# facebookresearch/pytorchvideo

Measured on NVIDIA H100. Metric: clips/sec forward (synthetic 3xTx224^2), higher is better.
Workload: dtype f16

## Files before the change

### pytorchvideo_b200/csrc/pv_epilogue.cuh

```cuda
#pragma once
#include "pv_common.cuh"
#include "pv_sm90.cuh"

namespace pv {
namespace sm90 {

constexpr int EPI_STAGING_BYTES = 2 * 128 * 128;
constexpr int EPI_THREADS = 256;
constexpr int EPI_BAR_ID = 1;
constexpr int MAX_BN = 128;

struct EpiParams {
  CUtensorMap y_map;
  CUtensorMap r_map;
  int block_n, Co, rows, act, has_residual;
  const __half* addend;
  long long add_n, add_t;
  int add_off;
  int o_ext[4], o_box[4], o_pos[4];
  int hw, To;
};

inline void epi_set_addend(EpiParams& E, const pv_conv3d_desc* d) {
  E.addend = static_cast<const __half*>(d->addend);
  E.add_n = d->add_n_stride;
  E.add_t = d->add_t_stride;
  E.add_off = d->add_ch_off;
  E.hw = d->Ho * d->Wo;
  E.To = d->To;
}

__device__ __forceinline__ void tma_store_5d(const void* tmap, uint32_t src, int c0, int c1, int c2, int c3,
                                             int c4) {
  asm volatile(
      "cp.async.bulk.tensor.5d.global.shared::cta.bulk_group [%0, {%2, %3, %4, %5, %6}], [%1];" ::"l"(
          reinterpret_cast<uint64_t>(tmap)),
      "r"(src), "r"(c0), "r"(c1), "r"(c2), "r"(c3), "r"(c4)
      : "memory");
}
__device__ __forceinline__ void tma_store_commit() { asm volatile("cp.async.bulk.commit_group;" ::: "memory"); }
__device__ __forceinline__ void tma_store_wait_read0() { asm volatile("cp.async.bulk.wait_group.read 0;" ::: "memory"); }
__device__ __forceinline__ void tma_store_wait_all() { asm volatile("cp.async.bulk.wait_group 0;" ::: "memory"); }
__device__ __forceinline__ void fence_proxy_async_smem() { asm volatile("fence.proxy.async.shared::cta;" ::: "memory"); }
__device__ __forceinline__ void epi_bar_sync(int id, int nthreads) {
  asm volatile("bar.sync %0, %1;" ::"r"(id), "r"(nthreads) : "memory");
}

template <int ACT>
__device__ __forceinline__ float act_t(float x) {
  if (ACT == PV_ACT_RELU) return fmaxf(x, 0.f);
  if (ACT == PV_ACT_NONE) return x;
  return apply_act(x, ACT);
}

__device__ __forceinline__ void epilogue_begin(const EpiParams& E, uint32_t staging, uint32_t res_bar, int n0, int c1,
                                               int c2, int c3, int c4) {
  tma_store_wait_read0();
  if (E.has_residual) {
    const int nsub = (E.block_n + 63) >> 6;
    mbar_arrive_expect_tx(res_bar, (uint32_t)(nsub * E.rows * 128));
    for (int s = 0; s < nsub; ++s)
      tma_load_5d(staging + (uint32_t)s * 16384u, &E.r_map, res_bar, n0 + s * 64, c1, c2, c3, c4);
  }
}

template <int BN, int ACT, bool RES>
__device__ __forceinline__ void epi_math(const float (&d)[BN / 2], uint8_t* stg, const float* __restrict__ scale,
                                         const float* __restrict__ bias, int Co, int n0, int ctid) {
  const int lane = ctid & 31;
  const int row0 = 64 * (ctid >> 7) + 16 * ((ctid >> 5) & 3) + (lane >> 2);
  const int cq = 2 * (lane & 3);
#pragma unroll
  for (int j = 0; j < BN / 8; ++j) {
    const int col = 8 * j + cq;
    const int c = n0 + col;
    float2 s = make_float2(0.f, 0.f), b = make_float2(0.f, 0.f);
    if (c < Co) {
      s = __ldg(reinterpret_cast<const float2*>(scale + c));
      b = __ldg(reinterpret_cast<const float2*>(bias + c));
    }
#pragma unroll
    for (int i = 0; i < 2; ++i) {
      const int row = row0 + 8 * i;
      __half2* cell = reinterpret_cast<__half2*>(stg + (col >> 6) * 16384 + row * 128 +
                                                 ((((col & 63) >> 3) ^ (row & 7)) << 4) + cq * 2);
      float f0 = fmaf(d[4 * j + 2 * i], s.x, b.x), f1 = fmaf(d[4 * j + 2 * i + 1], s.y, b.y);
// ... 30 lines not shown
      const unsigned v = (unsigned)(m == 0 ? c1 : m == 1 ? c2 : m == 2 ? c3 : c4) + r % (unsigned)E.o_box[m];
      r /= (unsigned)E.o_box[m];
      inside &= v < (unsigned)E.o_ext[m];
      pos += v * (unsigned)E.o_pos[m];
    }
    if (!inside) continue;
    const unsigned nt = pos / (unsigned)E.hw;
    const unsigned n = nt / (unsigned)E.To, t = nt - n * (unsigned)E.To;
    const uint4 av = __ldg(reinterpret_cast<const uint4*>(acol + n * E.add_n + t * E.add_t));
    uint4* cell = reinterpret_cast<uint4*>(stg + (col >> 6) * 16384 + row * 128 + ((((col & 63) >> 3) ^ (row & 7)) << 4));
    uint4 sv = *cell;
    __half2* s2 = reinterpret_cast<__half2*>(&sv);
    const __half2* a2 = reinterpret_cast<const __half2*>(&av);
#pragma unroll
    for (int k = 0; k < 4; ++k) {
      const float2 f = __half22float2(s2[k]), g = __half22float2(a2[k]);
      s2[k] = __floats2half2_rn(f.x + g.x, f.y + g.y);
    }
    *cell = sv;
  }
}

template <int BN>
__device__ __forceinline__ void epilogue_tile(const EpiParams& E, const float* __restrict__ scale,
                                              const float* __restrict__ bias, const float (&d)[BN / 2],
                                              uint32_t staging, uint8_t* staging_gen, uint32_t res_bar,
                                              uint32_t& res_phase, int ctid, int n0, int c1, int c2, int c3, int c4) {
  epi_bar_sync(EPI_BAR_ID, EPI_THREADS);
  if (E.has_residual) {
    mbar_wait(res_bar, res_phase);
    res_phase ^= 1u;
  }
  switch (E.act) {
    case PV_ACT_RELU: epi_math_res<BN, PV_ACT_RELU>(E.has_residual, d, staging_gen, scale, bias, E.Co, n0, ctid); break;
    case PV_ACT_NONE: epi_math_res<BN, PV_ACT_NONE>(E.has_residual, d, staging_gen, scale, bias, E.Co, n0, ctid); break;
    case PV_ACT_SWISH: epi_math_res<BN, PV_ACT_SWISH>(E.has_residual, d, staging_gen, scale, bias, E.Co, n0, ctid); break;
    case PV_ACT_GELU: epi_math_res<BN, PV_ACT_GELU>(E.has_residual, d, staging_gen, scale, bias, E.Co, n0, ctid); break;
    default: epi_math_res<BN, PV_ACT_SIGMOID>(E.has_residual, d, staging_gen, scale, bias, E.Co, n0, ctid); break;
  }
  if (E.addend) {
    epi_bar_sync(EPI_BAR_ID, EPI_THREADS);
    epi_addend<BN>(E, staging_gen, ctid, n0, c1, c2, c3, c4);
  }
  fence_proxy_async_smem();
  epi_bar_sync(EPI_BAR_ID, EPI_THREADS);
  if (ctid == 0) {
    const int nsub = (E.block_n + 63) >> 6;
    for (int s = 0; s < nsub; ++s) tma_store_5d(&E.y_map, staging + (uint32_t)s * 16384u, n0 + s * 64, c1, c2, c3, c4);
    tma_store_commit();
  }
}

__host__ __device__ inline int round_block_n(int co) { return co <= 16 ? 16 : (co <= 32 ? 32 : (co <= 64 ? 64 : 128)); }

}
}
```

### pytorchvideo_b200/csrc/pv_igemm.cu

```cuda
#include "pv_common.cuh"
#include "pv_sm90.cuh"
#include "pv_epilogue.cuh"

#include <mutex>
#include <stdlib.h>
#include <string.h>

namespace pv {

using namespace sm90;

constexpr int IG_BM = 128;
constexpr int IG_MAX_TAPS = 64;
constexpr int IG_MAX_MAPS = 8;
constexpr int IG_PROD_WARPS = 4;
constexpr int IG_CONS_WARPS = 8;
constexpr int IG_THREADS = (IG_CONS_WARPS + IG_PROD_WARPS) * 32;

struct IgemmParams {
  CUtensorMap a_maps[IG_MAX_MAPS];
  CUtensorMap b_map;
  int O[4];
  int box[4];
  int nt[4];
  int rows;
  int n_tiles, m_tiles;
  int block_n;
  int Co;
  int taps, num_kc;
  int kbytes;
  int stages;
  int G, cpt;
  int split_ab;
  EpiParams epi;
  signed char tap_q[IG_MAX_TAPS][4];
  unsigned char tap_map[IG_MAX_TAPS];
};

template <int BN, int KB, bool GROUPED>
__device__ __forceinline__ void igemm_body(const IgemmParams& P, const float* __restrict__ scale,
                                           const float* __restrict__ bias, int span_tiles) {
  extern __shared__ uint8_t smem_raw[];
  const uint32_t smem_base = (smem_u32(smem_raw) + 1023u) & ~1023u;
  uint8_t* smem_gen = smem_raw + (smem_base - smem_u32(smem_raw));
  const int stages = P.stages;
  constexpr int G = 128 / KB, K16 = KB / 32;
  const uint32_t a_bytes = (uint32_t)IG_BM * KB;
  const uint32_t b_bytes = (uint32_t)BN * KB;
  const uint32_t stage_bytes = (uint32_t)G * (a_bytes + b_bytes);
  constexpr int k_elems = KB / 2;
  const uint32_t staging_off = (uint32_t)((stages * stage_bytes + 1023u) & ~1023u);
  const uint32_t staging = smem_base + staging_off;
  const uint32_t bar_base = staging + (uint32_t)EPI_STAGING_BYTES;
  auto full_bar = [&](int s) { return bar_base + 8u * s; };
  auto empty_bar = [&](int s) { return bar_base + 8u * (stages + s); };
  const uint32_t res_bar = bar_base + 8u * (2 * stages);

  const int warp = threadIdx.x >> 5;
  const int lane = threadIdx.x & 31;

  if (threadIdx.x == 0) {
    prefetch_tmap(&P.b_map);
    prefetch_tmap(&P.a_maps[0]);
    prefetch_tmap(&P.epi.y_map);
    for (int s = 0; s < stages; ++s) {
      mbar_init(full_bar(s), 1);
      mbar_init(empty_bar(s), IG_CONS_WARPS);
    }
    mbar_init(res_bar, 1);
    fence_mbar_init();
  }
  __syncthreads();
  asm volatile("griddepcontrol.wait;" ::: "memory");
  asm volatile("griddepcontrol.launch_dependents;" ::: "memory");

  const int total_tiles = P.n_tiles * P.m_tiles;
  const int num_kb = P.taps * P.num_kc;
  auto tile_coords = [&](int tile, int& n_tile, int (&o)[4]) {
    n_tile = tile % P.n_tiles;
    int mt = tile / P.n_tiles;
#pragma unroll
    for (int i = 0; i < 4; ++i) { o[i] = (mt % P.nt[i]) * P.box[i]; mt /= P.nt[i]; }
  };

  if (warp >= IG_CONS_WARPS) {
    const int pw = warp - IG_CONS_WARPS;
    const int nsplit = P.split_ab;
    if (pw < nsplit) {
      int stage = 0;
      uint32_t phase = 0;
      const uint32_t tx_bytes = (uint32_t)P.rows * KB + b_bytes;
      const int num_kc = P.num_kc, cpt = P.cpt;
      for (int tile = blockIdx.x; tile < total_tiles; tile += gridDim.x) {
        int n_tile, o[4];
        tile_coords(tile, n_tile, o);
        const int n0 = n_tile * BN;
        const int c0 = GROUPED ? (n_tile / span_tiles) * num_kc * k_elems : 0;
        int tap = 0, kc = 0;
        for (int ch = 0; ch < cpt; ++ch) {
          const int kb0 = ch * G;
          const int nsub = min(G, num_kb - kb0);
          mbar_wait(empty_bar(stage), phase ^ 1u);
          const uint32_t st_base = smem_base + (uint32_t)stage * stage_bytes;
          if (elect_one()) {
            if (pw == 0) mbar_arrive_expect_tx(full_bar(stage), (uint32_t)G * tx_bytes);
            int tp = tap, kk = kc;
            for (int j = 0; j < G; ++j) {
              const bool pad = j >= nsub;
              const int t = pad ? P.taps - 1 : tp;
              if ((2 * j) % nsplit == pw) {
                const void* amap = &P.a_maps[P.tap_map[t]];
                tma_load_5d(st_base + (uint32_t)j * a_bytes, amap, full_bar(stage),
                            (pad ? num_kc * k_elems : kk * k_elems) + c0,
                            o[0] + P.tap_q[t][0], o[1] + P.tap_q[t][1], o[2] + P.tap_q[t][2], o[3] + P.tap_q[t][3]);
              }
              if ((2 * j + 1) % nsplit == pw)
                tma_load_2d(st_base + (uint32_t)G * a_bytes + (uint32_t)j * b_bytes, &P.b_map, full_bar(stage),
                            (kb0 + j) * k_elems, n0);
              if (++kk == num_kc) { kk = 0; ++tp; }
            }
          }
          __syncwarp();
          for (int j = 0; j < nsub; ++j) { if (++kc == num_kc) { kc = 0; ++tap; } }
          if (++stage == stages) { stage = 0; phase ^= 1u; }
        }
      }
    }
  } else {
    const int ctid = threadIdx.x;
    const uint32_t a_row_off = (uint32_t)(ctid >> 7) * 64u * (uint32_t)KB;
    const int cpt = P.cpt;
    int stage = 0;
    uint32_t phase = 0, res_phase = 0;
    float acc[BN / 2];
#pragma unroll
    for (int i = 0; i < BN / 2; ++i) acc[i] = 0.f;
    for (int tile = blockIdx.x; tile < total_tiles; tile += gridDim.x) {
      int n_tile, o[4];
      tile_coords(tile, n_tile, o);
      if (ctid == 0) epilogue_begin(P.epi, staging, res_bar, n_tile * BN, o[0], o[1], o[2], o[3]);
      int prev = -1;
      for (int ch = 0; ch < cpt; ++ch) {
        mbar_wait(full_bar(stage), phase);
        const uint32_t st_base = smem_base + (uint32_t)stage * stage_bytes;
        acc_fence(acc);
        wgmma_fence();
#pragma unroll
        for (int j = 0; j < G; ++j) {
          const uint64_t a_desc = make_kmajor_desc(st_base + (uint32_t)j * a_bytes + a_row_off, KB);
          const uint64_t b_desc = make_kmajor_desc(st_base + (uint32_t)G * a_bytes + (uint32_t)j * b_bytes, KB);
#pragma unroll
          for (int k = 0; k < K16; ++k) {
            Wgmma<BN>::mma(acc, a_desc + (uint64_t)(2 * k), b_desc + (uint64_t)(2 * k), (ch | j | k) != 0 ? 1u : 0u);
          }
        }
        wgmma_commit();
        acc_fence(acc);
        wgmma_wait<1>();
        mbar_arrive_if(empty_bar(prev < 0 ? stage : prev), prev >= 0 && lane == 0);
        prev = stage;
        if (++stage == stages) { stage = 0; phase ^= 1u; }
      }
      wgmma_wait<0>();
      acc_fence(acc);
      mbar_arrive_if(empty_bar(prev < 0 ? stage : prev), prev >= 0 && lane == 0);
      epilogue_tile<BN>(P.epi, scale, bias, acc, staging, smem_gen + staging_off, res_bar, res_phase, ctid, n_tile * BN,
                        o[0], o[1], o[2], o[3]);
    }
    if (ctid == 0) tma_store_wait_all();
  }
}

template <int BN, int KB>
__global__ void __launch_bounds__(IG_THREADS, 1)
conv3d_igemm_kernel(const __grid_constant__ IgemmParams P, const float* __restrict__ scale,
                    const float* __restrict__ bias) {
  igemm_body<BN, KB, false>(P, scale, bias, 1);
}

template <int BN, int KB>
__global__ void __launch_bounds__(IG_THREADS, 1)
conv3d_igemm_grouped_kernel(const __grid_constant__ IgemmParams P, const float* __restrict__ scale,
                            const float* __restrict__ bias, int span_tiles) {
  igemm_body<BN, KB, true>(P, scale, bias, span_tiles);
}

typedef CUresult (*EncodeTiledFn)(CUtensorMap*, CUtensorMapDataType, cuuint32_t, void*,
                                  const cuuint64_t*, const cuuint64_t*, const cuuint32_t*,
                                  const cuuint32_t*, CUtensorMapInterleave, CUtensorMapSwizzle,
                                  CUtensorMapL2promotion, CUtensorMapFloatOOBfill);

EncodeTiledFn get_encode_fn() {
// ... 197 lines not shown
      if (grouped && (c < 64 || span_n % c)) continue;
      if (c > round_block_n(co16)) continue;
      if (c < co16 && (c % 64)) continue;
      const long long tiles = (long long)P.m_tiles * cdiv(d->Co, c);
      const double waves = (double)cdiv(tiles, sm_count);
      const double cost = waves * tile_cycles(c) + 1e-3 * cdiv(d->Co, c);
      if (cost < best) { best = cost; bn = c; }
    }
    P.block_n = bn;
    P.n_tiles = (int)cdiv(d->Co, bn);
  }
  const bool wmode = window_mode(d);
  const bool narrow = conv3d_tma_narrow(d);
  const int win = wmode ? window_elems(d) : (narrow ? d->Ci : 64);
  P.kbytes = 2 * win;
  P.Co = d->Co;
  P.taps = wmode ? d->kt * d->kh : d->kt * d->kh * d->kw;
  P.num_kc = (wmode || narrow) ? 1 : d->ci_pad64 / 64;
  P.epi.block_n = P.block_n;
  P.epi.Co = d->Co;
  P.epi.rows = P.rows;
  P.epi.act = d->act;
  P.epi.has_residual = d->has_residual;
  epi_set_addend(P.epi, d);
  const int kb_bytes = (IG_BM + P.block_n) * P.kbytes;
  const size_t smem_fixed = 2048  + EPI_STAGING_BYTES + 16;
  {
    const int num_kb = P.taps * P.num_kc;
    const int G = 128 / P.kbytes;
    const int budget = (int)(227 * 1024 - smem_fixed) - 8 * (2 * 24 + 1);
    int st = budget / (G * kb_bytes);
    if (st > 24 / G) st = 24 / G > 2 ? 24 / G : 2;
    if (st < 2) st = 2;
    P.G = G;
    P.split_ab = G >= 2 ? 4 : 2;
    P.cpt = (num_kb + G - 1) / G;
    P.stages = st;
    if (grouped && (G != 1 || P.block_n > span_n || span_n % P.block_n)) {
      set_error("internal: grouped mode needs one k-block per stage and BLOCK_N | N_span (G=%d BN=%d N_span=%d)", G,
                P.block_n, span_n);
      return PV_ERR_INVALID;
    }
  }
  const int stage_bytes = P.G * kb_bytes;
  const size_t smem_bytes = (size_t)P.stages * stage_bytes + smem_fixed + 8 * (2 * P.stages + 1);

  int ks[4], ss[4], ps[4], dls[4];
  for (int i = 0; i < 4; ++i) { ks[i] = pl.dim[i].k; ss[i] = pl.dim[i].s; ps[i] = pl.dim[i].p; dls[i] = pl.dim[i].dil; }
  const int* orig2m = pl.orig2m;
  unsigned used_maps = 0;
  const int kw_loop = wmode ? 1 : d->kw;
  for (int it = 0; it < d->kt; ++it)
    for (int ih = 0; ih < d->kh; ++ih)
      for (int iw = 0; iw < kw_loop; ++iw) {
        const int tap = (it * d->kh + ih) * kw_loop + iw;
        int q[4] = {0, 0, 0, 0}, r[4] = {0, 0, 0, 0};
        const int offs[3] = {wmode ? 0 : iw * d->dw - d->pw, ih * d->dh - d->ph, it * d->dt - d->pt};
        const int strd[3] = {wmode ? 1 : d->sw, d->sh, d->st};
        for (int o = 0; o < 3; ++o) {
          const int m = orig2m[o];
          if (strd[o] == 1 && offs[o] == 0) continue;
          const int qq = floordiv(offs[o], strd[o]);
          q[m] = qq;
          r[m] = offs[o] - qq * strd[o];
        }
        int cls = 0, mul = 1;
        for (int m = 0; m < 4; ++m) { cls += r[m] * mul; mul *= ss[m]; }
        if (cls >= IG_MAX_MAPS) { set_error("internal: parity class %d", cls); return PV_ERR_INVALID; }
// ... 136 lines not shown
```

### pytorchvideo_b200/csrc/pv_igemm_gather.cu

```cuda
#include "pv_common.cuh"
#include "pv_sm90.cuh"
#include "pv_epilogue.cuh"

#include <mutex>
#include <stdlib.h>
#include <string.h>

namespace pv {

using namespace sm90;

constexpr int GG_BM = 128;
constexpr int GG_BK = 64;
constexpr int GG_A_BYTES = GG_BM * GG_BK * 2;
constexpr int GG_MAX_UNITS = 256;
constexpr int GG_CONS_WARPS = 8;
constexpr int GG_PROD_WARPS = 4;
constexpr int GG_THREADS = (GG_CONS_WARPS + GG_PROD_WARPS) * 32;

struct GatherParams {
  CUtensorMap b_map;
  int N, Ti, Hi, Wi, To, Ho, Wo;
  int st, sh, sw, pt, ph, pw;
  int gbytes;
  int units_total;
  int upk;
  int upt, taps;
  int num_kb;
  long long x_row_stride;
  long long M;
  int m_tiles, n_tiles, block_n, Co, stages;
  int nprod;
  int depth;
  EpiParams epi;
  int unit_off[GG_MAX_UNITS];
  unsigned int unit_d[GG_MAX_UNITS];
};

template <int BN>
__global__ void __launch_bounds__(GG_THREADS, 1)
conv3d_igemm_gather_kernel(const __grid_constant__ GatherParams P, const __half* __restrict__ x,
                           const float* __restrict__ scale, const float* __restrict__ bias) {
  extern __shared__ uint8_t smem_raw[];
  const uint32_t smem_base = (smem_u32(smem_raw) + 1023u) & ~1023u;
  uint8_t* smem_gen = smem_raw + (smem_base - smem_u32(smem_raw));
  const int stages = P.stages;
  const uint32_t b_bytes = (uint32_t)BN * GG_BK * 2;
  const uint32_t stage_bytes = GG_A_BYTES + b_bytes;
  const uint32_t staging_off = (uint32_t)((stages * stage_bytes + 1023u) & ~1023u);
  const uint32_t staging = smem_base + staging_off;
  const uint32_t bar_base = staging + (uint32_t)EPI_STAGING_BYTES;
  auto full_bar = [&](int s) { return bar_base + 8u * s; };
  auto empty_bar = [&](int s) { return bar_base + 8u * (stages + s); };
  const uint32_t res_bar = bar_base + 8u * (2 * stages);

  __shared__ int s_off[GG_MAX_UNITS];
  __shared__ unsigned s_d[GG_MAX_UNITS];
  for (int i = threadIdx.x; i < GG_MAX_UNITS; i += blockDim.x) { s_off[i] = P.unit_off[i]; s_d[i] = P.unit_d[i]; }
  const int warp = threadIdx.x >> 5;
  const int lane = threadIdx.x & 31;
  constexpr int PROD_WARP0 = GG_CONS_WARPS;

  if (threadIdx.x == 0) {
    prefetch_tmap(&P.b_map);
    prefetch_tmap(&P.epi.y_map);
    for (int s = 0; s < stages; ++s) {
      mbar_init(full_bar(s), 2);
      mbar_init(empty_bar(s), GG_CONS_WARPS);
    }
    mbar_init(res_bar, 1);
    fence_mbar_init();
  }
  __syncthreads();
  asm volatile("griddepcontrol.wait;" ::: "memory");
  asm volatile("griddepcontrol.launch_dependents;" ::: "memory");

  const int total_tiles = P.n_tiles * P.m_tiles;

  if (warp >= PROD_WARP0) {
    const int wprod = warp - PROD_WARP0;
    const int my_tiles = (total_tiles - (int)blockIdx.x + (int)gridDim.x - 1) / (int)gridDim.x;
    const int total_g = my_tiles * P.num_kb;
    int cur_seq = -1;
    const __half* xrow[4];
    unsigned long long vmask[4];
    int n_tile = 0;
    const unsigned Ti = (unsigned)P.Ti, Hi = (unsigned)P.Hi, Wi = (unsigned)P.Wi;
    const uint32_t rsw = (uint32_t)(lane & 7);
    const uint32_t row_off = (uint32_t)lane * 128u;
    const bool deep = P.depth >= 2;
    int pending = -1;
    for (int g = wprod; wprod < P.nprod && g < total_g; g += P.nprod) {
      const int tile_seq = g / P.num_kb;
      const int kb = g - tile_seq * P.num_kb;
      const int stage = g % stages;
      const uint32_t phase = (uint32_t)((g / stages) & 1);
      if (tile_seq != cur_seq) {
        cur_seq = tile_seq;
        const int tile = (int)blockIdx.x + tile_seq * (int)gridDim.x;
        n_tile = tile % P.n_tiles;
        const int m_tile = tile / P.n_tiles;
        int t0[4], h0[4], w0[4];
// ... 74 lines not shown
          fence_proxy_async_smem();
          __syncwarp();
          if (elect_one()) mbar_arrive(full_bar(pending));
          __syncwarp();
        }
        pending = stage;
      } else {
        asm volatile("cp.async.wait_group 0;" ::: "memory");
        fence_proxy_async_smem();
        __syncwarp();
        if (elect_one()) mbar_arrive(full_bar(stage));
      }
    }
    if (pending >= 0) {
      asm volatile("cp.async.wait_group 0;" ::: "memory");
      fence_proxy_async_smem();
      __syncwarp();
      if (elect_one()) mbar_arrive(full_bar(pending));
    }
  } else if (warp < GG_CONS_WARPS) {
    const int ctid = threadIdx.x;
    const uint32_t a_row_off = (uint32_t)(ctid >> 7) * 64u * 128u;
    const int num_kb = P.num_kb;
    int stage = 0;
    uint32_t phase = 0, res_phase = 0;
    float acc[BN / 2];
#pragma unroll
    for (int i = 0; i < BN / 2; ++i) acc[i] = 0.f;
    for (int tile = blockIdx.x; tile < total_tiles; tile += gridDim.x) {
      const int n_tile = tile % P.n_tiles;
      const int m_tile = tile / P.n_tiles;
      if (ctid == 0) epilogue_begin(P.epi, staging, res_bar, n_tile * BN, m_tile * GG_BM, 0, 0, 0);
      int prev = -1;
      for (int kb = 0; kb < num_kb; ++kb) {
        mbar_wait(full_bar(stage), phase);
        const uint32_t a_addr = smem_base + stage * stage_bytes;
        const uint64_t a_desc = make_kmajor_desc(a_addr + a_row_off, 128);
        const uint64_t b_desc = make_kmajor_desc(a_addr + GG_A_BYTES, 128);
        acc_fence(acc);
        wgmma_fence();
#pragma unroll
        for (int k = 0; k < GG_BK / 16; ++k)
          Wgmma<BN>::mma(acc, a_desc + (uint64_t)(2 * k), b_desc + (uint64_t)(2 * k), (kb | k) != 0 ? 1u : 0u);
        wgmma_commit();
        acc_fence(acc);
        wgmma_wait<1>();
        mbar_arrive_if(empty_bar(prev < 0 ? stage : prev), prev >= 0 && lane == 0);
        prev = stage;
        if (++stage == stages) { stage = 0; phase ^= 1u; }
      }
      wgmma_wait<0>();
      acc_fence(acc);
      mbar_arrive_if(empty_bar(prev < 0 ? stage : prev), prev >= 0 && lane == 0);
      epilogue_tile<BN>(P.epi, scale, bias, acc, staging, smem_gen + staging_off, res_bar, res_phase, ctid, n_tile * BN,
                        m_tile * GG_BM, 0, 0, 0);
    }
    if (ctid == 0) tma_store_wait_all();
  }
}

typedef CUresult (*EncodeTiledFn)(CUtensorMap*, CUtensorMapDataType, cuuint32_t, void*,
                                  const cuuint64_t*, const cuuint64_t*, const cuuint32_t*,
                                  const cuuint32_t*, CUtensorMapInterleave, CUtensorMapSwizzle,
                                  CUtensorMapL2promotion, CUtensorMapFloatOOBfill);
EncodeTiledFn get_encode_fn();

int conv3d_gather_supported(const pv_conv3d_desc* d) {
  if (d->dtype != PV_F16 || d->groups != 1) return 0;
  if (!(d->Ci == 4 || (d->Ci % 8 == 0 && d->Ci < 64))) return 0;
  if (d->Co % 8) return 0;
  if (d->ci_pad64 != d->Ci) return 0;
  const int gbytes = d->Ci == 4 ? 8 : 16;
  const int units = d->kt * d->kh * d->kw * (d->Ci * 2 / gbytes);
  if (units > GG_MAX_UNITS) return 0;
  if (d->x_row_stride % (gbytes / 2) || d->y_row_stride % 8 || (d->has_residual && d->res_row_stride % 8)) return 0;
  if (d->dt * (d->kt - 1) > 255 || d->dh * (d->kh - 1) > 255 || d->dw * (d->kw - 1) > 255) return 0;
  if (d->kt * d->kh * d->kw > 64) return 0;
  const long long M = (long long)d->N * d->To * d->Ho * d->Wo;
  if (M >= (1ll << 31)) return 0;
  return 1;
// ... 30 lines not shown
        const int tap = (it * d->kh + ih) * d->kw + iw;
        const int dt = it * d->dt, dh = ih * d->dh, dw = iw * d->dw;
        const long long off = (((long long)dt * d->Hi + dh) * d->Wi + dw) * d->x_row_stride;
        for (int q = 0; q < upt; ++q) {
          const int u = tap * upt + q;
          const long long o = off + (long long)q * (P.gbytes / 2);
          if (o > 0x7fffffffll) { set_error("gather offset overflow"); return PV_ERR_UNSUPPORTED; }
          P.unit_off[u] = (int)o;
          P.unit_d[u] = (unsigned)dt | ((unsigned)dh << 8) | ((unsigned)dw << 16) | ((unsigned)tap << 24);
        }
      }
  {
    const int co16 = (int)cdiv(d->Co, 16) * 16;
    int bn = round_block_n(co16);
    while (bn > 64 && (long long)P.m_tiles * cdiv(d->Co, bn) < 2 * sm_count && (bn / 2) % 64 == 0) bn /= 2;
    P.block_n = bn;
    P.n_tiles = (int)cdiv(d->Co, bn);
  }
  P.epi.block_n = P.block_n;
  P.epi.Co = d->Co;
  P.epi.rows = GG_BM;
  P.epi.act = d->act;
  P.epi.has_residual = d->has_residual;
  epi_set_addend(P.epi, d);
  for (int m = 0; m < 4; ++m) {
    P.epi.o_ext[m] = m == 0 ? (int)P.M : 1;
    P.epi.o_box[m] = m == 0 ? GG_BM : 1;
    P.epi.o_pos[m] = m == 0 ? 1 : 0;
  }
  const int stage_bytes = GG_A_BYTES + P.block_n * GG_BK * 2;
  {
    int st = (227 * 1024 - 2048 - 2048  - EPI_STAGING_BYTES - 512) / stage_bytes;
    if (st > 16) st = 16;
    if (st < 2) { set_error("gather: not enough smem stages"); return PV_ERR_UNSUPPORTED; }
    static const bool shallow = getenv("PVB200_GATHER_DEPTH2") == nullptr;
    P.nprod = st < GG_PROD_WARPS ? st : GG_PROD_WARPS;
    if (!shallow && st >= 8 && st / 2 < P.nprod) P.nprod = st / 2;
    P.stages = (st / P.nprod) * P.nprod;
    P.depth = (!shallow && P.stages >= 2 * P.nprod) ? 2 : 1;
  }
  const size_t smem_bytes = (size_t)P.stages * stage_bytes + 2048 + EPI_STAGING_BYTES + 8 * (2 * P.stages + 1) + 16;
  for (int pass = 0; pass < 2; ++pass) {
    if (pass == 1 && !d->has_residual) break;
    const long long rs = pass == 0 ? d->y_row_stride : d->res_row_stride;
    void* base = pass == 0 ? y : const_cast<void*>(residual);
    cuuint64_t gdim[5] = {(cuuint64_t)d->Co, (cuuint64_t)P.M, 1, 1, 1};
    cuuint64_t gstr[4] = {(cuuint64_t)rs * 2, (cuuint64_t)rs * 2 * (cuuint64_t)P.M, (cuuint64_t)rs * 2 * (cuuint64_t)P.M,
                          (cuuint64_t)rs * 2 * (cuuint64_t)P.M};
    cuuint32_t box[5] = {64, GG_BM, 1, 1, 1}, estr[5] = {1, 1, 1, 1, 1};
    CUresult cr = encode(pass == 0 ? &P.epi.y_map : &P.epi.r_map, CU_TENSOR_MAP_DATA_TYPE_FLOAT16, 5, base, gdim, gstr,
                         box, estr, CU_TENSOR_MAP_INTERLEAVE_NONE, CU_TENSOR_MAP_SWIZZLE_128B,
                         CU_TENSOR_MAP_L2_PROMOTION_L2_128B, CU_TENSOR_MAP_FLOAT_OOB_FILL_NONE);
    if (cr != CUDA_SUCCESS) { set_error("cuTensorMapEncodeTiled(gather %s) failed: %d", pass ? "R" : "Y", (int)cr); return PV_ERR_CUDA; }
  }
  {
    const long long kpad = (long long)cdiv((long long)taps * d->Ci, 64) * 64;
    cuuint64_t gdim[2] = {(cuuint64_t)kpad, (cuuint64_t)d->Co};
    cuuint64_t gstr[1] = {(cuuint64_t)kpad * 2};
    cuuint32_t box[2] = {64, (cuuint32_t)P.block_n}, estr[2] = {1, 1};
    CUresult cr = encode(&P.b_map, CU_TENSOR_MAP_DATA_TYPE_FLOAT16, 2, (void*)w, gdim, gstr, box, estr,
                         CU_TENSOR_MAP_INTERLEAVE_NONE, CU_TENSOR_MAP_SWIZZLE_128B,
                         CU_TENSOR_MAP_L2_PROMOTION_L2_256B, CU_TENSOR_MAP_FLOAT_OOB_FILL_NONE);
    if (cr != CUDA_SUCCESS) { set_error("cuTensorMapEncodeTiled(B, gather) failed: %d", (int)cr); return PV_ERR_CUDA; }
  }
// ... 34 lines not shown
```

### pytorchvideo_b200/csrc/pv_stem.cu

```cuda
#include "pv_common.cuh"
#include "pv_sm90.cuh"
#include "pv_epilogue.cuh"

#include <stdlib.h>
#include <string.h>

namespace pv {

using namespace sm90;

typedef CUresult (*EncodeTiledFn)(CUtensorMap*, CUtensorMapDataType, cuuint32_t, void*,
                                  const cuuint64_t*, const cuuint64_t*, const cuuint32_t*,
                                  const cuuint32_t*, CUtensorMapInterleave, CUtensorMapSwizzle,
                                  CUtensorMapL2promotion, CUtensorMapFloatOOBfill);
EncodeTiledFn get_encode_fn();

constexpr int ST_CONS_WARPS = 8;
constexpr int ST_PROD_WARPS = 4;
constexpr int ST_THREADS = (ST_CONS_WARPS + ST_PROD_WARPS) * 32;
constexpr int ST_MAX_ROWS = 64;

struct StemParams {
  int N, Ti, Hi, To, Ho, Wo;
  int kt, kh, st, sh, pt, ph, dt, dh;
  int rows;
  int win;
  int wtiles;
  int n16;
  int stages;
  unsigned seg_bytes;
  unsigned w_bytes;
  long long row_pitch;
  long long base_off;
  EpiParams epi;
};

__device__ __forceinline__ void bulk_g2s(uint32_t dst, const void* src, uint32_t bytes, uint32_t bar) {
  asm volatile("cp.async.bulk.shared::cluster.global.mbarrier::complete_tx::bytes [%0], [%1], %2, [%3];" ::"r"(dst),
               "l"(src), "r"(bytes), "r"(bar)
               : "memory");
}
template <int BN, int KS>
__global__ void __launch_bounds__(ST_THREADS, 1)
conv3d_stem_rows_kernel(const __grid_constant__ StemParams P, const unsigned char* __restrict__ x,
                        const unsigned char* __restrict__ w, const unsigned char* __restrict__ zero_row,
                        const float* __restrict__ scale, const float* __restrict__ bias) {
  extern __shared__ uint8_t smem_raw[];
  const uint32_t smem_base = (smem_u32(smem_raw) + 1023u) & ~1023u;
  uint8_t* smem_gen = smem_raw + (smem_base - smem_u32(smem_raw));
  const int stages = P.stages;
  const uint32_t w_off = 0;
  const uint32_t ring_off = (P.w_bytes + 1023u) & ~1023u;
  const uint32_t stage_bytes = (uint32_t)P.rows * P.seg_bytes + 2048u;
  const uint32_t staging_off = (ring_off + (uint32_t)stages * stage_bytes + 1023u) & ~1023u;
  const uint32_t staging = smem_base + staging_off;
  const uint32_t bar_base = staging + (uint32_t)EPI_STAGING_BYTES;
  auto full_bar = [&](int s) { return bar_base + 8u * s; };
  auto empty_bar = [&](int s) { return bar_base + 8u * (stages + s); };
  const uint32_t res_bar = bar_base + 8u * (2 * stages);
  const uint32_t w_bar = res_bar + 8u;

  const int warp = threadIdx.x >> 5, lane = threadIdx.x & 31;
  if (threadIdx.x == 0) {
    for (int s = 0; s < stages; ++s) { mbar_init(full_bar(s), 1); mbar_init(empty_bar(s), ST_CONS_WARPS); }
    mbar_init(res_bar, 1);
    mbar_init(w_bar, 1);
    prefetch_tmap(&P.epi.y_map);
    fence_mbar_init();
  }
  __syncthreads();
  asm volatile("griddepcontrol.wait;" ::: "memory");
  asm volatile("griddepcontrol.launch_dependents;" ::: "memory");

  const int total_tiles = P.N * P.To * P.Ho * P.wtiles;
  auto tile_coords = [&](int tile, int& wt, int& ho, int& to, int& n) {
    wt = tile % P.wtiles; tile /= P.wtiles;
    ho = tile % P.Ho; tile /= P.Ho;
    to = tile % P.To; n = tile / P.To;
  };

  if (warp >= ST_CONS_WARPS) {
    const int pw = warp - ST_CONS_WARPS;
    if (pw == 0 && elect_one()) {
      mbar_arrive_expect_tx(w_bar, P.w_bytes);
      for (uint32_t o = 0; o < P.w_bytes; o += 32768u)
        bulk_g2s(smem_base + w_off + o, w + o, min(32768u, P.w_bytes - o), w_bar);
    }
    int stage = 0;
    uint32_t phase = 0;
    const long long frame_pitch = P.row_pitch * P.Hi;
    for (int tile = blockIdx.x; tile < total_tiles; tile += gridDim.x) {
      int wt, ho, to, n;
      tile_coords(tile, wt, ho, to, n);
      mbar_wait(empty_bar(stage), phase ^ 1u);
      const uint32_t st_base = smem_base + ring_off + (uint32_t)stage * stage_bytes;
      const long long col0 = P.base_off + (long long)wt * 128 * 16;
      long long want = 127ll * 16 + (long long)P.win * 2;
      if (col0 + want > P.row_pitch) want = P.row_pitch - col0;
      const uint32_t nbytes = (uint32_t)want;
      if (elect_one()) {
        if (pw == 0) mbar_arrive_expect_tx(full_bar(stage), (uint32_t)P.rows * nbytes);
        for (int r = pw; r < P.rows; r += ST_PROD_WARPS) {
          const int fdt = r / P.kh, fdh = r - fdt * P.kh;
          const int ti = to * P.st - P.pt + fdt * P.dt, hi = ho * P.sh - P.ph + fdh * P.dh;
          const bool ok = (unsigned)ti < (unsigned)P.Ti && (unsigned)hi < (unsigned)P.Hi;
          const unsigned char* src = ok ? x + ((long long)n * P.Ti + ti) * frame_pitch + (long long)hi * P.row_pitch + col0
                                        : zero_row;
          bulk_g2s(st_base + (uint32_t)r * P.seg_bytes, src, nbytes, full_bar(stage));
        }
      }
      __syncwarp();
      if (++stage == stages) { stage = 0; phase ^= 1u; }
    }
  } else {
    const int ctid = threadIdx.x;
    const uint32_t a_row_off = (uint32_t)(ctid >> 7) * 64u * 16u;
    const uint32_t b_lbo = (uint32_t)P.n16 * 16u;
    int stage = 0;
    uint32_t phase = 0, res_phase = 0;
    float acc[BN / 2];
#pragma unroll
    for (int i = 0; i < BN / 2; ++i) acc[i] = 0.f;
    mbar_wait(w_bar, 0);
    for (int tile = blockIdx.x; tile < total_tiles; tile += gridDim.x) {
      int wt, ho, to, n;
      tile_coords(tile, wt, ho, to, n);
      if (ctid == 0) epilogue_begin(P.epi, staging, res_bar, 0, wt * 128, ho, to, n);
      mbar_wait(full_bar(stage), phase);
      const uint32_t st_base = smem_base + ring_off + (uint32_t)stage * stage_bytes;
#pragma unroll 1
      for (int r = 0; r < P.rows; ++r) {
        acc_fence(acc);
        wgmma_fence();
#pragma unroll
        for (int ks = 0; ks < KS; ++ks) {
          const uint64_t a_desc = make_noswz_desc(st_base + (uint32_t)r * P.seg_bytes + (uint32_t)ks * 32u + a_row_off, 16u, 128u);
          const uint64_t b_desc = make_noswz_desc(smem_base + w_off + (uint32_t)((r * P.win + ks * 16) >> 3) * b_lbo, b_lbo, 128u);
          Wgmma<BN>::mma(acc, a_desc, b_desc, (r | ks) != 0 ? 1u : 0u);
        }
        wgmma_commit();
        acc_fence(acc);
        wgmma_wait<1>();
      }
      wgmma_wait<0>();
      acc_fence(acc);
      mbar_arrive_if(empty_bar(stage), lane == 0);
      if (++stage == stages) { stage = 0; phase ^= 1u; }
      epilogue_tile<BN>(P.epi, scale, bias, acc, staging, smem_gen + staging_off, res_bar, res_phase, ctid, 0, wt * 128, ho,
                        to, n);
    }
    if (ctid == 0) tma_store_wait_all();
  }
}

static int stem_window_lead(const pv_conv3d_desc* d) { return (((d->x_w_pad - d->pw) * d->Ci * 2) % 16) ? 1 : 0; }

}

using namespace pv;

extern "C" int pv_conv3d_stem_rows_supported(const pv_conv3d_desc* d) {
  if (!d || d->dtype != PV_F16 || d->groups != 1 || d->has_residual) return 0;
  if (d->Ci != 4 || d->sw != 2 || d->dw != 1 || d->x_w_pad <= 0 || d->x_row_stride != 4) return 0;
  if (d->x_w_pad < d->pw || (d->x_w_phys * 8) % 16) return 0;
  const int lead = stem_window_lead(d);
  const int run = (d->kw + lead) * 4;
  const int win = run <= 16 ? 16 : (run <= 32 ? 32 : 64);
  if (run > 64 || d->ci_pad64 != win) return 0;
  if (d->Co % 8 || d->Co > MAX_BN || d->y_row_stride % 8) return 0;
  if (d->kt * d->kh > ST_MAX_ROWS) return 0;
  if (!conv3d_addend_ok(d)) return 0;
  const long long base_off = (long long)(d->x_w_pad - d->pw - lead) * 8;
  if (base_off < 0 || base_off % 16) return 0;
  if (base_off + (long long)(d->Wo - 1) * 16 + (long long)win * 2 > (long long)d->x_w_phys * 8) return 0;
// ... 4 lines not shown
}

extern "C" int pv_conv3d_stem_rows_fwd(const pv_conv3d_desc* d, const void* x, const void* w, const float* scale,
                                       const float* bias, const void* zero_row, void* y, void* stream) {
  PV_CHECK_ARG(d && x && w && scale && bias && zero_row && y, "null argument");
  if (!pv_conv3d_stem_rows_supported(d)) { set_error("stem rows kernel: unsupported convolution"); return PV_ERR_UNSUPPORTED; }
  EncodeTiledFn encode = get_encode_fn();
  if (!encode) { set_error("cuTensorMapEncodeTiled entry point unavailable"); return PV_ERR_CUDA; }
  const int sm_count = current_sm_count();
  if (sm_count <= 0) { set_error("cannot query the SM count"); return PV_ERR_CUDA; }
  StemParams P;
  memset(&P, 0, sizeof(P));
  P.N = d->N; P.Ti = d->Ti; P.Hi = d->Hi; P.To = d->To; P.Ho = d->Ho; P.Wo = d->Wo;
  P.kt = d->kt; P.kh = d->kh; P.st = d->st; P.sh = d->sh; P.pt = d->pt; P.ph = d->ph; P.dt = d->dt; P.dh = d->dh;
  P.rows = d->kt * d->kh;
  P.win = d->ci_pad64;
  P.wtiles = (int)cdiv(d->Wo, 128);
  P.n16 = (d->Co + 15) / 16 * 16;
  const int block_n = round_block_n(P.n16);
  P.row_pitch = (long long)d->x_w_phys * 8;
  P.base_off = (long long)(d->x_w_pad - d->pw - stem_window_lead(d)) * 8;
  P.w_bytes = (unsigned)((long long)P.rows * P.win * P.n16 * 2);
  P.seg_bytes = (unsigned)((127 * 16 + P.win * 2 + 127) & ~127);
  const size_t smem_fixed = 2048 + ((P.w_bytes + 1023) & ~1023u) + 1024 + EPI_STAGING_BYTES + 8 * (2 * 8 + 2) + 16;
  const unsigned stage_bytes = (unsigned)P.rows * P.seg_bytes + 2048u;
  {
    const long long budget = 227 * 1024 - (long long)smem_fixed;
    long long st = budget / stage_bytes;
    if (st > 8) st = 8;
    if (st < 2) { set_error("stem rows kernel: not enough shared memory for two stages"); return PV_ERR_UNSUPPORTED; }
    P.stages = (int)st;
  }
  const size_t smem_bytes = smem_fixed + (size_t)P.stages * stage_bytes;
  P.epi.block_n = block_n;
  P.epi.Co = d->Co;
  P.epi.rows = d->Wo < 128 ? d->Wo : 128;
  P.epi.act = d->act;
  P.epi.has_residual = 0;
  const long long ostr[4] = {1, d->Wo, (long long)d->Wo * d->Ho, (long long)d->Wo * d->Ho * d->To};
  const int O[4] = {d->Wo, d->Ho, d->To, d->N};
  const int box[4] = {P.epi.rows, 1, 1, 1};
  epi_set_addend(P.epi, d);
  for (int m = 0; m < 4; ++m) {
    P.epi.o_ext[m] = O[m];
    P.epi.o_box[m] = box[m];
    P.epi.o_pos[m] = (int)ostr[m];
  }
  {
// ... 44 lines not shown
```

Before: 1719.

## Move epilogue TMA stores and residual loads to dedicated DMA warp with double-buffered staging

Adds a dedicated epilogue DMA warp that issues residual TMA loads and output TMA stores. Staging is double-buffered and coordinated through ready/full mbarriers, replacing the named-barrier syncs and the single-thread store issue inside the consumer warpgroups. Consumers can now start the next tile's math while the previous tile's store drains, at the cost of more shared memory for staging (fewer pipeline stages possible) and one fewer producer warp in some kernels.

```diff
diff --git a/pytorchvideo_b200/csrc/pv_epilogue.cuh b/pytorchvideo_b200/csrc/pv_epilogue.cuh
--- a/pytorchvideo_b200/csrc/pv_epilogue.cuh
+++ b/pytorchvideo_b200/csrc/pv_epilogue.cuh
@@ -6,14 +6,19 @@
 namespace sm90 {
 
 constexpr int EPI_STAGING_BYTES = 2 * 128 * 128;
+constexpr int EPI_MAX_BUFS = 2;
+constexpr int EPI_BARS = 2 * EPI_MAX_BUFS;
 constexpr int EPI_THREADS = 256;
 constexpr int EPI_BAR_ID = 1;
 constexpr int MAX_BN = 128;
+
+constexpr int epi_smem_bytes(int nbuf) { return nbuf * EPI_STAGING_BYTES + 8 * EPI_BARS; }
 
 struct EpiParams {
   CUtensorMap y_map;
   CUtensorMap r_map;
   int block_n, Co, rows, act, has_residual;
+  int nbuf;
   const __half* addend;
   long long add_n, add_t;
   int add_off;
@@ -53,15 +58,57 @@
   return apply_act(x, ACT);
 }
 
-__device__ __forceinline__ void epilogue_begin(const EpiParams& E, uint32_t staging, uint32_t res_bar, int n0, int c1,
-                                               int c2, int c3, int c4) {
-  tma_store_wait_read0();
-  if (E.has_residual) {
-    const int nsub = (E.block_n + 63) >> 6;
-    mbar_arrive_expect_tx(res_bar, (uint32_t)(nsub * E.rows * 128));
+struct EpiSmem {
+  uint32_t staging;
+  uint8_t* staging_gen;
+  uint32_t bars;
+  __device__ __forceinline__ uint32_t buf(int b) const { return staging + (uint32_t)b * EPI_STAGING_BYTES; }
+  __device__ __forceinline__ uint8_t* buf_gen(int b) const { return staging_gen + b * EPI_STAGING_BYTES; }
+  __device__ __forceinline__ uint32_t ready(int b) const { return bars + 8u * b; }
+  __device__ __forceinline__ uint32_t full(int b) const { return bars + 8u * (EPI_MAX_BUFS + b); }
+  __device__ __forceinline__ void init() const {
+    for (int b = 0; b < EPI_MAX_BUFS; ++b) {
+      mbar_init(ready(b), 1);
+      mbar_init(full(b), EPI_THREADS / 32);
+    }
+  }
+};
+
+template <class Coords>
+__device__ __forceinline__ void epilogue_dma(const EpiParams& E, const EpiSmem& S, int total_tiles, Coords coords) {
+  if (!elect_one()) return;
+  const int nbuf = E.nbuf;
+  const int nsub = (E.block_n + 63) >> 6;
+  auto fill = [&](int tile, int b) {
+    if (E.has_residual) {
+      int n0, c[4];
+      coords(tile, n0, c);
+      mbar_arrive_expect_tx(S.ready(b), (uint32_t)(nsub * E.rows * 128));
+      for (int s = 0; s < nsub; ++s)
+        tma_load_5d(S.buf(b) + (uint32_t)s * 16384u, &E.r_map, S.ready(b), n0 + s * 64, c[0], c[1], c[2], c[3]);
+    } else {
+      mbar_arrive(S.ready(b));
+    }
+  };
+  for (int b = 0; b < nbuf; ++b) {
+    const int tile = (int)blockIdx.x + b * (int)gridDim.x;
+    if (tile < total_tiles) fill(tile, b);
+  }
+  int b = 0;
+  uint32_t phase = 0;
+  for (int tile = blockIdx.x; tile < total_tiles; tile += gridDim.x) {
+    mbar_wait(S.full(b), phase);
+    int n0, c[4];
+    coords(tile, n0, c);
     for (int s = 0; s < nsub; ++s)
-      tma_load_5d(staging + (uint32_t)s * 16384u, &E.r_map, res_bar, n0 + s * 64, c1, c2, c3, c4);
-  }
+      tma_store_5d(&E.y_map, S.buf(b) + (uint32_t)s * 16384u, n0 + s * 64, c[0], c[1], c[2], c[3]);
+    tma_store_commit();
+    tma_store_wait_read0();
+    const long long next = (long long)tile + (long long)nbuf * gridDim.x;
+    if (next < total_tiles) fill((int)next, b);
+    if (++b == nbuf) { b = 0; phase ^= 1u; }
+  }
+  tma_store_wait_all();
 }
 
 template <int BN, int ACT, bool RES>
@@ -138,15 +185,12 @@
 }
 
 template <int BN>
-__device__ __forceinline__ void epilogue_tile(const EpiParams& E, const float* __restrict__ scale,
-                                              const float* __restrict__ bias, const float (&d)[BN / 2],
-                                              uint32_t staging, uint8_t* staging_gen, uint32_t res_bar,
-                                              uint32_t& res_phase, int ctid, int n0, int c1, int c2, int c3, int c4) {
-  epi_bar_sync(EPI_BAR_ID, EPI_THREADS);
-  if (E.has_residual) {
-    mbar_wait(res_bar, res_phase);
-    res_phase ^= 1u;
-  }
+__device__ __forceinline__ void epilogue_tile(const EpiParams& E, const EpiSmem& S, int& buf, uint32_t& phase,
+                                              const float* __restrict__ scale, const float* __restrict__ bias,
+                                              const float (&d)[BN / 2], int ctid, int n0, int c1, int c2, int c3,
+                                              int c4) {
+  mbar_wait(S.ready(buf), phase);
+  uint8_t* staging_gen = S.buf_gen(buf);
   switch (E.act) {
     case PV_ACT_RELU: epi_math_res<BN, PV_ACT_RELU>(E.has_residual, d, staging_gen, scale, bias, E.Co, n0, ctid); break;
     case PV_ACT_NONE: epi_math_res<BN, PV_ACT_NONE>(E.has_residual, d, staging_gen, scale, bias, E.Co, n0, ctid); break;
@@ -159,12 +203,9 @@
     epi_addend<BN>(E, staging_gen, ctid, n0, c1, c2, c3, c4);
   }
   fence_proxy_async_smem();
-  epi_bar_sync(EPI_BAR_ID, EPI_THREADS);
-  if (ctid == 0) {
-    const int nsub = (E.block_n + 63) >> 6;
-    for (int s = 0; s < nsub; ++s) tma_store_5d(&E.y_map, staging + (uint32_t)s * 16384u, n0 + s * 64, c1, c2, c3, c4);
-    tma_store_commit();
-  }
+  __syncwarp();
+  mbar_arrive_if(S.full(buf), (ctid & 31) == 0);
+  if (++buf == E.nbuf) { buf = 0; phase ^= 1u; }
 }
 
 __host__ __device__ inline int round_block_n(int co) { return co <= 16 ? 16 : (co <= 32 ? 32 : (co <= 64 ? 64 : 128)); }
diff --git a/pytorchvideo_b200/csrc/pv_igemm.cu b/pytorchvideo_b200/csrc/pv_igemm.cu
--- a/pytorchvideo_b200/csrc/pv_igemm.cu
+++ b/pytorchvideo_b200/csrc/pv_igemm.cu
@@ -16,6 +16,7 @@
 constexpr int IG_PROD_WARPS = 4;
 constexpr int IG_CONS_WARPS = 8;
 constexpr int IG_THREADS = (IG_CONS_WARPS + IG_PROD_WARPS) * 32;
+constexpr int IG_DMA_WARP = IG_CONS_WARPS + IG_PROD_WARPS - 1;
 
 struct IgemmParams {
   CUtensorMap a_maps[IG_MAX_MAPS];
@@ -51,10 +52,10 @@
   constexpr int k_elems = KB / 2;
   const uint32_t staging_off = (uint32_t)((stages * stage_bytes + 1023u) & ~1023u);
   const uint32_t staging = smem_base + staging_off;
-  const uint32_t bar_base = staging + (uint32_t)EPI_STAGING_BYTES;
+  const uint32_t bar_base = staging + (uint32_t)(P.epi.nbuf * EPI_STAGING_BYTES);
   auto full_bar = [&](int s) { return bar_base + 8u * s; };
   auto empty_bar = [&](int s) { return bar_base + 8u * (stages + s); };
-  const uint32_t res_bar = bar_base + 8u * (2 * stages);
+  const EpiSmem epi{staging, smem_gen + staging_off, bar_base + 8u * (2 * stages)};
 
   const int warp = threadIdx.x >> 5;
   const int lane = threadIdx.x & 31;
@@ -67,7 +68,7 @@
       mbar_init(full_bar(s), 1);
       mbar_init(empty_bar(s), IG_CONS_WARPS);
     }
-    mbar_init(res_bar, 1);
+    epi.init();
     fence_mbar_init();
   }
   __syncthreads();
@@ -83,7 +84,13 @@
     for (int i = 0; i < 4; ++i) { o[i] = (mt % P.nt[i]) * P.box[i]; mt /= P.nt[i]; }
   };
 
-  if (warp >= IG_CONS_WARPS) {
+  if (warp == IG_DMA_WARP) {
+    epilogue_dma(P.epi, epi, total_tiles, [&](int tile, int& n0, int (&c)[4]) {
+      int n_tile;
+      tile_coords(tile, n_tile, c);
+      n0 = n_tile * BN;
+    });
+  } else if (warp >= IG_CONS_WARPS) {
     const int pw = warp - IG_CONS_WARPS;
     const int nsplit = P.split_ab;
     if (pw < nsplit) {
@@ -130,15 +137,14 @@
     const int ctid = threadIdx.x;
     const uint32_t a_row_off = (uint32_t)(ctid >> 7) * 64u * (uint32_t)KB;
     const int cpt = P.cpt;
-    int stage = 0;
-    uint32_t phase = 0, res_phase = 0;
+    int stage = 0, epi_buf = 0;
+    uint32_t phase = 0, epi_phase = 0;
     float acc[BN / 2];
 #pragma unroll
     for (int i = 0; i < BN / 2; ++i) acc[i] = 0.f;
     for (int tile = blockIdx.x; tile < total_tiles; tile += gridDim.x) {
       int n_tile, o[4];
       tile_coords(tile, n_tile, o);
-      if (ctid == 0) epilogue_begin(P.epi, staging, res_bar, n_tile * BN, o[0], o[1], o[2], o[3]);
       int prev = -1;
       for (int ch = 0; ch < cpt; ++ch) {
         mbar_wait(full_bar(stage), phase);
@@ -164,10 +170,8 @@
       wgmma_wait<0>();
       acc_fence(acc);
       mbar_arrive_if(empty_bar(prev < 0 ? stage : prev), prev >= 0 && lane == 0);
-      epilogue_tile<BN>(P.epi, scale, bias, acc, staging, smem_gen + staging_off, res_bar, res_phase, ctid, n_tile * BN,
-                        o[0], o[1], o[2], o[3]);
-    }
-    if (ctid == 0) tma_store_wait_all();
+      epilogue_tile<BN>(P.epi, epi, epi_buf, epi_phase, scale, bias, acc, ctid, n_tile * BN, o[0], o[1], o[2], o[3]);
+    }
   }
 }
 
@@ -411,18 +415,19 @@
   P.epi.rows = P.rows;
   P.epi.act = d->act;
   P.epi.has_residual = d->has_residual;
+  P.epi.nbuf = EPI_MAX_BUFS;
   epi_set_addend(P.epi, d);
   const int kb_bytes = (IG_BM + P.block_n) * P.kbytes;
-  const size_t smem_fixed = 2048  + EPI_STAGING_BYTES + 16;
+  const size_t smem_fixed = 2048  + epi_smem_bytes(P.epi.nbuf) + 16;
   {
     const int num_kb = P.taps * P.num_kc;
     const int G = 128 / P.kbytes;
-    const int budget = (int)(227 * 1024 - smem_fixed) - 8 * (2 * 24 + 1);
+    const int budget = (int)(227 * 1024 - smem_fixed) - 8 * (2 * 24);
     int st = budget / (G * kb_bytes);
     if (st > 24 / G) st = 24 / G > 2 ? 24 / G : 2;
     if (st < 2) st = 2;
     P.G = G;
-    P.split_ab = G >= 2 ? 4 : 2;
+    P.split_ab = G >= 2 ? 3 : 2;
     P.cpt = (num_kb + G - 1) / G;
     P.stages = st;
     if (grouped && (G != 1 || P.block_n > span_n || span_n % P.block_n)) {
@@ -432,7 +437,7 @@
     }
   }
   const int stage_bytes = P.G * kb_bytes;
-  const size_t smem_bytes = (size_t)P.stages * stage_bytes + smem_fixed + 8 * (2 * P.stages + 1);
+  const size_t smem_bytes = (size_t)P.stages * stage_bytes + smem_fixed + 8 * (2 * P.stages);
 
   int ks[4], ss[4], ps[4], dls[4];
   for (int i = 0; i < 4; ++i) { ks[i] = pl.dim[i].k; ss[i] = pl.dim[i].s; ps[i] = pl.dim[i].p; dls[i] = pl.dim[i].dil; }
diff --git a/pytorchvideo_b200/csrc/pv_igemm_gather.cu b/pytorchvideo_b200/csrc/pv_igemm_gather.cu
--- a/pytorchvideo_b200/csrc/pv_igemm_gather.cu
+++ b/pytorchvideo_b200/csrc/pv_igemm_gather.cu
@@ -15,8 +15,9 @@
 constexpr int GG_A_BYTES = GG_BM * GG_BK * 2;
 constexpr int GG_MAX_UNITS = 256;
 constexpr int GG_CONS_WARPS = 8;
-constexpr int GG_PROD_WARPS = 4;
-constexpr int GG_THREADS = (GG_CONS_WARPS + GG_PROD_WARPS) * 32;
+constexpr int GG_PROD_WARPS = 3;
+constexpr int GG_THREADS = (GG_CONS_WARPS + GG_PROD_WARPS + 1) * 32;
+constexpr int GG_DMA_WARP = GG_CONS_WARPS + GG_PROD_WARPS;
 
 struct GatherParams {
   CUtensorMap b_map;
@@ -49,10 +50,10 @@
   const uint32_t stage_bytes = GG_A_BYTES + b_bytes;
   const uint32_t staging_off = (uint32_t)((stages * stage_bytes + 1023u) & ~1023u);
   const uint32_t staging = smem_base + staging_off;
-  const uint32_t bar_base = staging + (uint32_t)EPI_STAGING_BYTES;
+  const uint32_t bar_base = staging + (uint32_t)(P.epi.nbuf * EPI_STAGING_BYTES);
   auto full_bar = [&](int s) { return bar_base + 8u * s; };
   auto empty_bar = [&](int s) { return bar_base + 8u * (stages + s); };
-  const uint32_t res_bar = bar_base + 8u * (2 * stages);
+  const EpiSmem epi{staging, smem_gen + staging_off, bar_base + 8u * (2 * stages)};
 
   __shared__ int s_off[GG_MAX_UNITS];
   __shared__ unsigned s_d[GG_MAX_UNITS];
@@ -68,7 +69,7 @@
       mbar_init(full_bar(s), 2);
       mbar_init(empty_bar(s), GG_CONS_WARPS);
     }
-    mbar_init(res_bar, 1);
+    epi.init();
     fence_mbar_init();
   }
   __syncthreads();
@@ -77,7 +78,13 @@
 
   const int total_tiles = P.n_tiles * P.m_tiles;
 
-  if (warp >= PROD_WARP0) {
+  if (warp == GG_DMA_WARP) {
+    epilogue_dma(P.epi, epi, total_tiles, [&](int tile, int& n0, int (&c)[4]) {
+      n0 = (tile % P.n_tiles) * BN;
+      c[0] = (tile / P.n_tiles) * GG_BM;
+      c[1] = c[2] = c[3] = 0;
+    });
+  } else if (warp >= PROD_WARP0) {
     const int wprod = warp - PROD_WARP0;
     const int my_tiles = (total_tiles - (int)blockIdx.x + (int)gridDim.x - 1) / (int)gridDim.x;
     const int total_g = my_tiles * P.num_kb;
@@ -198,15 +205,14 @@
     const int ctid = threadIdx.x;
     const uint32_t a_row_off = (uint32_t)(ctid >> 7) * 64u * 128u;
     const int num_kb = P.num_kb;
-    int stage = 0;
-    uint32_t phase = 0, res_phase = 0;
+    int stage = 0, epi_buf = 0;
+    uint32_t phase = 0, epi_phase = 0;
     float acc[BN / 2];
 #pragma unroll
     for (int i = 0; i < BN / 2; ++i) acc[i] = 0.f;
     for (int tile = blockIdx.x; tile < total_tiles; tile += gridDim.x) {
       const int n_tile = tile % P.n_tiles;
       const int m_tile = tile / P.n_tiles;
-      if (ctid == 0) epilogue_begin(P.epi, staging, res_bar, n_tile * BN, m_tile * GG_BM, 0, 0, 0);
       int prev = -1;
       for (int kb = 0; kb < num_kb; ++kb) {
         mbar_wait(full_bar(stage), phase);
@@ -228,10 +234,8 @@
       wgmma_wait<0>();
       acc_fence(acc);
       mbar_arrive_if(empty_bar(prev < 0 ? stage : prev), prev >= 0 && lane == 0);
-      epilogue_tile<BN>(P.epi, scale, bias, acc, staging, smem_gen + staging_off, res_bar, res_phase, ctid, n_tile * BN,
-                        m_tile * GG_BM, 0, 0, 0);
-    }
-    if (ctid == 0) tma_store_wait_all();
+      epilogue_tile<BN>(P.epi, epi, epi_buf, epi_phase, scale, bias, acc, ctid, n_tile * BN, m_tile * GG_BM, 0, 0, 0);
+    }
   }
 }
 
@@ -308,6 +312,7 @@
   P.epi.rows = GG_BM;
   P.epi.act = d->act;
   P.epi.has_residual = d->has_residual;
+  P.epi.nbuf = EPI_MAX_BUFS;
   epi_set_addend(P.epi, d);
   for (int m = 0; m < 4; ++m) {
     P.epi.o_ext[m] = m == 0 ? (int)P.M : 1;
@@ -316,16 +321,15 @@
   }
   const int stage_bytes = GG_A_BYTES + P.block_n * GG_BK * 2;
   {
-    int st = (227 * 1024 - 2048 - 2048  - EPI_STAGING_BYTES - 512) / stage_bytes;
+    int st = (227 * 1024 - 2048 - 2048  - epi_smem_bytes(P.epi.nbuf) - 512) / stage_bytes;
     if (st > 16) st = 16;
     if (st < 2) { set_error("gather: not enough smem stages"); return PV_ERR_UNSUPPORTED; }
     static const bool shallow = getenv("PVB200_GATHER_DEPTH2") == nullptr;
     P.nprod = st < GG_PROD_WARPS ? st : GG_PROD_WARPS;
-    if (!shallow && st >= 8 && st / 2 < P.nprod) P.nprod = st / 2;
-    P.stages = (st / P.nprod) * P.nprod;
+    P.stages = st;
     P.depth = (!shallow && P.stages >= 2 * P.nprod) ? 2 : 1;
   }
-  const size_t smem_bytes = (size_t)P.stages * stage_bytes + 2048 + EPI_STAGING_BYTES + 8 * (2 * P.stages + 1) + 16;
+  const size_t smem_bytes = (size_t)P.stages * stage_bytes + 2048 + epi_smem_bytes(P.epi.nbuf) + 8 * (2 * P.stages) + 16;
   for (int pass = 0; pass < 2; ++pass) {
     if (pass == 1 && !d->has_residual) break;
     const long long rs = pass == 0 ? d->y_row_stride : d->res_row_stride;
diff --git a/pytorchvideo_b200/csrc/pv_stem.cu b/pytorchvideo_b200/csrc/pv_stem.cu
--- a/pytorchvideo_b200/csrc/pv_stem.cu
+++ b/pytorchvideo_b200/csrc/pv_stem.cu
@@ -16,8 +16,9 @@
 EncodeTiledFn get_encode_fn();
 
 constexpr int ST_CONS_WARPS = 8;
-constexpr int ST_PROD_WARPS = 4;
-constexpr int ST_THREADS = (ST_CONS_WARPS + ST_PROD_WARPS) * 32;
+constexpr int ST_PROD_WARPS = 3;
+constexpr int ST_THREADS = (ST_CONS_WARPS + ST_PROD_WARPS + 1) * 32;
+constexpr int ST_DMA_WARP = ST_CONS_WARPS + ST_PROD_WARPS;
 constexpr int ST_MAX_ROWS = 64;
 
 struct StemParams {
@@ -54,16 +55,16 @@
   const uint32_t stage_bytes = (uint32_t)P.rows * P.seg_bytes + 2048u;
   const uint32_t staging_off = (ring_off + (uint32_t)stages * stage_bytes + 1023u) & ~1023u;
   const uint32_t staging = smem_base + staging_off;
-  const uint32_t bar_base = staging + (uint32_t)EPI_STAGING_BYTES;
+  const uint32_t bar_base = staging + (uint32_t)(P.epi.nbuf * EPI_STAGING_BYTES);
   auto full_bar = [&](int s) { return bar_base + 8u * s; };
   auto empty_bar = [&](int s) { return bar_base + 8u * (stages + s); };
-  const uint32_t res_bar = bar_base + 8u * (2 * stages);
-  const uint32_t w_bar = res_bar + 8u;
+  const EpiSmem epi{staging, smem_gen + staging_off, bar_base + 8u * (2 * stages)};
+  const uint32_t w_bar = epi.bars + 8u * EPI_BARS;
 
   const int warp = threadIdx.x >> 5, lane = threadIdx.x & 31;
   if (threadIdx.x == 0) {
     for (int s = 0; s < stages; ++s) { mbar_init(full_bar(s), 1); mbar_init(empty_bar(s), ST_CONS_WARPS); }
-    mbar_init(res_bar, 1);
+    epi.init();
     mbar_init(w_bar, 1);
     prefetch_tmap(&P.epi.y_map);
     fence_mbar_init();
@@ -79,7 +80,13 @@
     to = tile % P.To; n = tile / P.To;
   };
 
-  if (warp >= ST_CONS_WARPS) {
+  if (warp == ST_DMA_WARP) {
+    epilogue_dma(P.epi, epi, total_tiles, [&](int tile, int& n0, int (&c)[4]) {
+      n0 = 0;
+      tile_coords(tile, c[0], c[1], c[2], c[3]);
+      c[0] *= 128;
+    });
+  } else if (warp >= ST_CONS_WARPS) {
     const int pw = warp - ST_CONS_WARPS;
     if (pw == 0 && elect_one()) {
       mbar_arrive_expect_tx(w_bar, P.w_bytes);
@@ -116,8 +123,8 @@
     const int ctid = threadIdx.x;
     const uint32_t a_row_off = (uint32_t)(ctid >> 7) * 64u * 16u;
     const uint32_t b_lbo = (uint32_t)P.n16 * 16u;
-    int stage = 0;
-    uint32_t phase = 0, res_phase = 0;
+    int stage = 0, epi_buf = 0;
+    uint32_t phase = 0, epi_phase = 0;
     float acc[BN / 2];
 #pragma unroll
     for (int i = 0; i < BN / 2; ++i) acc[i] = 0.f;
@@ -125,7 +132,6 @@
     for (int tile = blockIdx.x; tile < total_tiles; tile += gridDim.x) {
       int wt, ho, to, n;
       tile_coords(tile, wt, ho, to, n);
-      if (ctid == 0) epilogue_begin(P.epi, staging, res_bar, 0, wt * 128, ho, to, n);
       mbar_wait(full_bar(stage), phase);
       const uint32_t st_base = smem_base + ring_off + (uint32_t)stage * stage_bytes;
 #pragma unroll 1
@@ -146,10 +152,8 @@
       acc_fence(acc);
       mbar_arrive_if(empty_bar(stage), lane == 0);
       if (++stage == stages) { stage = 0; phase ^= 1u; }
-      epilogue_tile<BN>(P.epi, scale, bias, acc, staging, smem_gen + staging_off, res_bar, res_phase, ctid, 0, wt * 128, ho,
-                        to, n);
+      epilogue_tile<BN>(P.epi, epi, epi_buf, epi_phase, scale, bias, acc, ctid, 0, wt * 128, ho, to, n);
     }
-    if (ctid == 0) tma_store_wait_all();
   }
 }
 
@@ -200,8 +204,13 @@
   P.base_off = (long long)(d->x_w_pad - d->pw - stem_window_lead(d)) * 8;
   P.w_bytes = (unsigned)((long long)P.rows * P.win * P.n16 * 2);
   P.seg_bytes = (unsigned)((127 * 16 + P.win * 2 + 127) & ~127);
-  const size_t smem_fixed = 2048 + ((P.w_bytes + 1023) & ~1023u) + 1024 + EPI_STAGING_BYTES + 8 * (2 * 8 + 2) + 16;
   const unsigned stage_bytes = (unsigned)P.rows * P.seg_bytes + 2048u;
+  size_t smem_fixed = 0;
+  for (int nbuf = EPI_MAX_BUFS; nbuf >= 1; --nbuf) {
+    P.epi.nbuf = nbuf;
+    smem_fixed = 2048 + ((P.w_bytes + 1023) & ~1023u) + 1024 + epi_smem_bytes(nbuf) + 8 * (2 * 8 + 1) + 16;
+    if (227 * 1024 - (long long)smem_fixed >= 2ll * stage_bytes) break;
+  }
   {
     const long long budget = 227 * 1024 - (long long)smem_fixed;
     long long st = budget / stage_bytes;
```

After: 1783 (median of 6 runs). 3.7% higher.
